# fateshelled/onnx_image_processing

Hardware: AMD Instinct MI355X
Metric: image-pairs/sec (640x480, K=512) (higher is better)
Workload: dtype f32; 1 GPU; Shi-Tomasi(3) + NMS(r=5)/top-k + sparse BAD(512, hard) + Sinkhorn(20, eps 0.05) + MNN(100, 0.1), 640x480 gray pairs, K=512 (BASELINE configs[1]); height=480, width=640, max_keypoints=512, parallelism=pair-sharded x1, input=float32 frames resident in HBM

## Files before the change

onnx_image_processing_amd/csrc/bad.hip:

```cpp
#include "common.h"

#include <math.h>

#include <memory>
#include <mutex>
#include <type_traits>
#include <vector>

#include "bad_plan_opt.h"

namespace {

constexpr int WIN = 34;
constexpr int WOFF = 16;
constexpr int SP = WIN + 1;
constexpr int FR = 33;
constexpr int FW = 35;

struct BadPlan {
  int geometry_ok;
  int num_pairs;
  int passes;
  int passes_canonical;
};
// ... 136 lines not shown
    for (int g = 0; g < GMAX; ++g) {
      if (g < groups) {
        const uint32_t q = plan_geom[g * 64 + lane];
        const int tint = plan_tint[g * 64 + lane];
        const int rad = (int)((q >> 20) & 15u);
        auto box = [&](int offx, int offy) {
          const int cx = clampi((int)kx + offx, 0, w - 1) - ox, cy = clampi((int)ky + offy, 0, h - 1) - oy;
          const int a = cy - rad, b = cy + rad + 1, l = cx - rad, r = cx + rad + 1;
          return (isat[b * FW + r] - isat[a * FW + r]) - (isat[b * FW + l] - isat[a * FW + l]);
        };
        const int s1 = box((int)(q & 31u) - 16, (int)((q >> 10) & 31u) - 16);
        const int s2 = box((int)((q >> 5) & 31u) - 16, (int)((q >> 15) & 31u) - 16);
        emit(g, s1 - s2, tint);
      }
    }
  }
  if (bits) {
    unsigned long long mine = 0ull;
#pragma unroll
    for (int g = 0; g < GMAX; ++g) mine = (lane == g) ? wordv[g] : mine;
    if (lane < groups) reinterpret_cast<unsigned long long *>(bits + (size_t)flat * words)[lane] = mine;
  }
  if (desc) {
    const float inv = normalize ? fmaxf(sqrtf((float)pop), 1e-12f) : 1.0f;
#pragma unroll
    for (int g = 0; g < GMAX; ++g) {
      if (g < groups) {
        const float v = ((wordv[g] >> lane) & 1ull) ? 1.0f : 0.0f;
        desc[(size_t)flat * num_pairs + g * 64 + lane] = normalize ? v / inv : v;
      }
    }
  }
  if (lane == 0) status[flat] = 1;
}

template <typename PIX>
__global__ __launch_bounds__(64) void sparse_bad_kernel(MiSets images, int h, int w,
                                                        MiSets kpt_sets, int k, int total,
                                                        const uint32_t *__restrict__ geom,
                                                        const float *__restrict__ thr, int num_pairs,
                                                        int mode, float temperature, int normalize,
                                                        float scale_y, float scale_x,
                                                        float *__restrict__ desc,
                                                        uint32_t *__restrict__ bits,
                                                        const uint8_t *__restrict__ status, int chunk) {
  __shared__ double sat[SP * SP];
  __shared__ float vals[1024];
  const int lane = threadIdx.x;
  const int groups = num_pairs / 64;
  const int words = num_pairs / 32;

  unsigned long long todo = 1ull;
  int first = (int)xcd_contiguous_id(blockIdx.x, gridDim.x);
  if (status) {
    first = (int)blockIdx.x * chunk;
    const int mine = first + lane;
    todo = __ballot(lane < chunk && mine < total && status[mine] == 0);
    if (!todo) return;
  }
  uint32_t qg[8];
  float tg[8];
#pragma unroll
  for (int g = 0; g < 8; ++g) {
    qg[g] = (g < groups) ? geom[g * 64 + lane] : 0u;
    tg[g] = (g < groups) ? thr[g * 64 + lane] : 0.0f;
  }

  while (todo) {
    const int bit = __ffsll((long long)todo) - 1;
    todo &= todo - 1ull;
    const int flat = first + bit;
    const int img = flat / k;
    const PIX *im = mi_set_item<PIX>(images, img, (size_t)h * w);
    const float *kp = mi_set_item<float>(kpt_sets, img, (size_t)k * 2) + (size_t)(flat - img * k) * 2;
    const float ky_raw = kp[0];
    const float kx_raw = kp[1];
    const bool valid = ky_raw >= 0.0f;
    const float ky = fminf(fmaxf(ky_raw, 0.0f), (float)(h - 1));
    const float kx = fminf(fmaxf(kx_raw, 0.0f), (float)(w - 1));
    const int oy = (int)floorf(ky) - WOFF, ox = (int)floorf(kx) - WOFF;

    __syncthreads();
    for (int i = lane; i < SP; i += 64) { sat[i] = 0.0; sat[i * SP] = 0.0; }
    if (lane < WIN) {
      const int gx = clampi(ox + lane, 0, w - 1);
      PIX px[WIN];
#pragma unroll
      for (int r = 0; r < WIN; ++r) px[r] = im[(size_t)clampi(oy + r, 0, h - 1) * w + gx];
      double acc = 0.0;
#pragma unroll
      for (int r = 0; r < WIN; ++r) {
        acc += (double)px[r];
        sat[(r + 1) * SP + (lane + 1)] = acc;
      }
    }
    __syncthreads();
    if (lane < WIN) {
      double *row = sat + (lane + 1) * SP + 1;
      double v[WIN];
#pragma unroll
      for (int c = 0; c < WIN; ++c) v[c] = row[c];
      double acc = 0.0;
#pragma unroll
      for (int c = 0; c < WIN; ++c) { acc += v[c]; row[c] = acc; }
    }
    __syncthreads();

    const size_t drow = (size_t)flat * (size_t)num_pairs;
    uint32_t *brow = bits ? bits + (size_t)flat * words : nullptr;
    int pop = 0;
    float sumsq = 0.0f;
    auto eval_group = [&](int g, uint32_t q, float thr_p) {
      const int p = g * 64 + lane;
      const int x1 = (int)(q & 31u) - 16, x2 = (int)((q >> 5) & 31u) - 16;
      const int y1 = (int)((q >> 10) & 31u) - 16, y2 = (int)((q >> 15) & 31u) - 16;
      const int r = (int)((q >> 20) & 15u);
      const int c1y = nearest_centre(ky + (float)y1, scale_y, h) - oy;
      const int c1x = nearest_centre(kx + (float)x1, scale_x, w) - ox;
      const int c2y = nearest_centre(ky + (float)y2, scale_y, h) - oy;
      const int c2x = nearest_centre(kx + (float)x2, scale_x, w) - ox;
      const int a1 = clampi(c1y - r, 0, WIN), b1 = clampi(c1y + r + 1, 0, WIN);
      const int l1 = clampi(c1x - r, 0, WIN), r1 = clampi(c1x + r + 1, 0, WIN);
      const int a2 = clampi(c2y - r, 0, WIN), b2 = clampi(c2y + r + 1, 0, WIN);
      const int l2 = clampi(c2x - r, 0, WIN), r2 = clampi(c2x + r + 1, 0, WIN);
      const double s1 = (sat[b1 * SP + r1] - sat[a1 * SP + r1]) - (sat[b1 * SP + l1] - sat[a1 * SP + l1]);
      const double s2 = (sat[b2 * SP + r2] - sat[a2 * SP + r2]) - (sat[b2 * SP + l2] - sat[a2 * SP + l2]);
      const double area = (double)((2 * r + 1) * (2 * r + 1));
      const double t = (double)thr_p;
      if (mode == MI_BAD_HARD) {
        const bool bitv = valid && ((s1 - s2) <= t * area);
        const unsigned long long word = __ballot(bitv);
        pop += (int)__popcll(word);
        if (brow && lane == 0) {
          brow[2 * g] = (uint32_t)word;
          brow[2 * g + 1] = (uint32_t)(word >> 32);
        }
        if (desc) vals[p] = bitv ? 1.0f : 0.0f;
      } else {
        const float c = (float)((s1 - s2) / area - t);
        float v = c;
        if (mode == MI_BAD_SOFT) v = 1.0f / (1.0f + expf(c * temperature));
        v = valid ? v : 0.0f;
        sumsq += v * v;
        vals[p] = v;
      }
    };
#pragma unroll
    for (int g = 0; g < 8; ++g)
      if (g < groups) eval_group(g, qg[g], tg[g]);
#pragma unroll 1
    for (int g = 8; g < groups; ++g) eval_group(g, geom[g * 64 + lane], thr[g * 64 + lane]);

    if (desc) {
      float inv = 1.0f;
      if (normalize) {
        const float ss = (mode == MI_BAD_HARD) ? (float)pop : wave_sum(sumsq);
        inv = fmaxf(sqrtf(ss), 1e-12f);
      }
      for (int g = 0; g < groups; ++g) {
        const float v = vals[g * 64 + lane];
        desc[drow + g * 64 + lane] = normalize ? v / inv : v;
      }
    }
  }
}

struct HostPlan {
  std::vector<uint32_t> geom;
  bool geometry_ok = false;
  mi::BadGatherSchedule sched;
};

std::vector<uint16_t> table_corners(const std::vector<uint32_t> &geom, bool *all_inside) {
  const int num_pairs = (int)geom.size();
  std::vector<uint16_t> c((size_t)num_pairs * 8);
  bool ok = true;
  auto word = [](int row, int col) { return (uint16_t)(row * FW + col); };
  for (int p = 0; p < num_pairs; ++p) {
    const uint32_t q = geom[p];
    const int x1 = (int)(q & 31u), x2 = (int)((q >> 5) & 31u);
    const int y1 = (int)((q >> 10) & 31u), y2 = (int)((q >> 15) & 31u);
    const int r = (int)((q >> 20) & 15u);
    const bool in = x1 - r >= 0 && x2 - r >= 0 && y1 - r >= 0 && y2 - r >= 0 && x1 + r <= 31 && x2 + r <= 31 &&
                    y1 + r <= 31 && y2 + r <= 31;
    ok = ok && in;
    const int cx1 = in ? x1 : 16, cy1 = in ? y1 : 16, cx2 = in ? x2 : 16, cy2 = in ? y2 : 16, cr = in ? r : 0;
    uint16_t *pos = &c[(size_t)p * 8], *neg = pos + 4;
    pos[0] = word(cy1 + cr + 1, cx1 + cr + 1);
    pos[1] = word(cy1 - cr, cx1 - cr);
    pos[2] = word(cy2 - cr, cx2 + cr + 1);
    pos[3] = word(cy2 + cr + 1, cx2 - cr);
    neg[0] = word(cy1 - cr, cx1 + cr + 1);
    neg[1] = word(cy1 + cr + 1, cx1 - cr);
    neg[2] = word(cy2 + cr + 1, cx2 + cr + 1);
    neg[3] = word(cy2 - cr, cx2 - cr);
  }
  *all_inside = ok;
  return c;
}

std::shared_ptr<const HostPlan> host_plan_for(const std::vector<uint32_t> &geom) {
  static std::mutex mu;
  static std::vector<std::shared_ptr<const HostPlan>> *cache = new std::vector<std::shared_ptr<const HostPlan>>();
  {
    std::lock_guard<std::mutex> lock(mu);
    for (const auto &hp : *cache)
      if (hp->geom == geom) return hp;
  }
  auto hp = std::make_shared<HostPlan>();
  hp->geom = geom;
  const std::vector<uint16_t> corners = table_corners(geom, &hp->geometry_ok);
  hp->sched = mi::schedule_bad_gathers(corners, (int)geom.size());
  std::lock_guard<std::mutex> lock(mu);
  if (cache->size() >= 16) cache->erase(cache->begin());
  cache->push_back(hp);
  return hp;
}

}

extern "C" size_t mi_bad_plan_bytes(int num_pairs) {
  if (num_pairs <= 0) return 0;
  return sizeof(BadPlan) + (size_t)num_pairs * (sizeof(uint4) + sizeof(int) + sizeof(uint32_t)) +
         (size_t)(num_pairs / 64) * (num_pairs / 64) * sizeof(uint64_t);
}

int mi_bad_plan_passes_host(const uint32_t *pair_geom_host, int num_pairs, int *canonical, int *scheduled) {
  if (!pair_geom_host || !canonical || !scheduled) return MI_E_NULL;
  if (num_pairs <= 0 || num_pairs % 64 != 0 || num_pairs > 1024) return MI_E_PARAM;
  const auto hp = host_plan_for(std::vector<uint32_t>(pair_geom_host, pair_geom_host + num_pairs));
  for (int e = 0; e < num_pairs; ++e)
    if (hp->sched.exec_pair[e] % 64 != e % 64) return MI_E_PARAM;
  *canonical = hp->sched.passes_canonical;
  *scheduled = hp->sched.passes;
  return MI_OK;
}

extern "C" int mi_bad_plan_build(const uint32_t *pair_geom, const float *pair_thr, int num_pairs, void *plan,
                                 mi_stream_t stream) {
  MI_ENTER();
  if (!pair_geom || !pair_thr || !plan) return MI_E_NULL;
  if (num_pairs <= 0 || num_pairs % 64 != 0 || num_pairs > 1024) return MI_E_PARAM;
  if (((uintptr_t)plan % 16) != 0) return MI_E_ALIGN;
  hipStream_t s = (hipStream_t)stream;
  std::vector<uint32_t> geom(num_pairs);
  std::vector<float> thr(num_pairs);
  if (hipMemcpyAsync(geom.data(), pair_geom, sizeof(uint32_t) * num_pairs, hipMemcpyDeviceToHost, s) != hipSuccess ||
      hipMemcpyAsync(thr.data(), pair_thr, sizeof(float) * num_pairs, hipMemcpyDeviceToHost, s) != hipSuccess ||
      hipStreamSynchronize(s) != hipSuccess)
    return mi_launch_status() ? mi_launch_status() : MI_E_PARAM;
  const auto sched = host_plan_for(geom);
  std::vector<char> host(mi_bad_plan_bytes(num_pairs));
  BadPlan *hp = reinterpret_cast<BadPlan *>(host.data());
  uint4 *offs = reinterpret_cast<uint4 *>(hp + 1);
  int *tint = reinterpret_cast<int *>(offs + num_pairs);
  uint32_t *xgeom = reinterpret_cast<uint32_t *>(tint + num_pairs);
  uint64_t *masks = reinterpret_cast<uint64_t *>(xgeom + num_pairs);
  const int rounds = num_pairs / 64;
  for (int i = 0; i < rounds * rounds; ++i) masks[i] = 0;
  for (int e = 0; e < num_pairs; ++e) {
    const int p = sched->sched.exec_pair[e], lane = e % 64, round = e / 64;
    const uint16_t *pos = &sched->sched.pos[(size_t)e * 4], *neg = &sched->sched.neg[(size_t)e * 4];
    auto two = [](uint16_t lo, uint16_t hi) { return (uint32_t)(lo * 4u) | ((uint32_t)(hi * 4u) << 16); };
    offs[e] = make_uint4(two(pos[0], pos[1]), two(pos[2], pos[3]), two(neg[0], neg[1]), two(neg[2], neg[3]));
    const int r = (int)((geom[p] >> 20) & 15u);
    tint[e] = (int)floor((double)thr[p] * (double)((2 * r + 1) * (2 * r + 1)));
    xgeom[e] = geom[p];
    masks[round * rounds + p / 64] |= (uint64_t)1 << lane;
  }
  hp->geometry_ok = sched->geometry_ok ? 1 : 0;
  hp->num_pairs = num_pairs;
  hp->passes = sched->sched.passes;
  hp->passes_canonical = sched->sched.passes_canonical;
  if (hipMemcpyAsync(plan, host.data(), host.size(), hipMemcpyHostToDevice, s) != hipSuccess ||
      hipStreamSynchronize(s) != hipSuccess)
    return mi_launch_status() ? mi_launch_status() : MI_E_PARAM;
  return MI_OK;
}

namespace {
template <typename PIX>
int sparse_bad_launch(MiSets image, int n, int h, int w, MiSets keypoints, int k, const uint32_t *pair_geom,
                      const float *pair_thr, int num_pairs, int mode, float temperature, int normalize, float *desc,
                      uint32_t *bits, const void *plan, uint8_t *status, mi_stream_t stream) {
  if (!image.a || !keypoints.a || !pair_geom || !pair_thr) return MI_E_NULL;
  if ((image.per_set < n && !image.b) || (keypoints.per_set < n && !keypoints.b)) return MI_E_NULL;
  if (!desc && !bits) return MI_E_NULL;
  if (n <= 0 || h <= 0 || w <= 0 || k <= 0) return MI_E_SHAPE;
  if (num_pairs <= 0 || num_pairs % 64 != 0 || num_pairs > 1024) return MI_E_PARAM;
  if (mode != MI_BAD_RAW && mode != MI_BAD_SOFT && mode != MI_BAD_HARD) return MI_E_PARAM;
  if (bits && mode != MI_BAD_HARD) return MI_E_PARAM;
  if ((long long)n * k > 0x7fffffffLL) return MI_E_SHAPE;
  hipStream_t s = (hipStream_t)stream;
  const int total = n * k;
  const float scale_y = (float)(2.0 / ((double)(h - 1) + 1e-8));
  const float scale_x = (float)(2.0 / ((double)(w - 1) + 1e-8));
  const bool fast = plan != nullptr && status != nullptr && mode == MI_BAD_HARD && h >= 32 && w >= 32 &&
                    (long long)h * w < (1LL << 30);
  if (fast) {
    const BadPlan *bp = reinterpret_cast<const BadPlan *>(plan);
    auto fast_kernel = num_pairs == 512 ? bad_fast_kernel<8, PIX> : num_pairs == 256 ? bad_fast_kernel<4, PIX> : bad_fast_kernel<0, PIX>;
    hipLaunchKernelGGL(fast_kernel, dim3((unsigned)ceil_div(total, 4)), dim3(256), 0, s, image, h, w, keypoints,
                       k, total, num_pairs, normalize, bp, pair_geom, desc, bits, status);
    constexpr int CHUNK = 16;
    hipLaunchKernelGGL(sparse_bad_kernel<PIX>, dim3((unsigned)ceil_div(total, CHUNK)), dim3(64), 0, s, image, h, w,
                       keypoints, k, total, pair_geom, pair_thr, num_pairs, mode, temperature, normalize, scale_y,
                       scale_x, desc, bits, status, CHUNK);
  } else {
    hipLaunchKernelGGL(sparse_bad_kernel<PIX>, dim3((unsigned)total), dim3(64), 0, s, image, h, w, keypoints, k, total,
                       pair_geom, pair_thr, num_pairs, mode, temperature, normalize, scale_y, scale_x, desc, bits,
                       nullptr, 1);
  }
  return mi_launch_status();
}
}

int mi_sparse_bad_sets(MiSets images, int pix_u8, int n, int h, int w, MiSets keypoints, int k, const uint32_t *pair_geom,
                       const float *pair_thr, int num_pairs, int mode, float temperature, int normalize, float *desc,
                       uint32_t *bits, const void *plan, uint8_t *status, mi_stream_t stream) {
  if (pix_u8)
    return sparse_bad_launch<uint8_t>(images, n, h, w, keypoints, k, pair_geom, pair_thr, num_pairs, mode, temperature,
                                      normalize, desc, bits, plan, status, stream);
  return sparse_bad_launch<float>(images, n, h, w, keypoints, k, pair_geom, pair_thr, num_pairs, mode, temperature,
                                  normalize, desc, bits, plan, status, stream);
}

extern "C" int mi_sparse_bad(const float *image, int n, int h, int w, const float *keypoints, int k,
                             const uint32_t *pair_geom, const float *pair_thr, int num_pairs, int mode,
                             float temperature, int normalize, float *desc, uint32_t *bits, const void *plan,
                             uint8_t *status, mi_stream_t stream) {
  MI_ENTER();
  return sparse_bad_launch<float>(mi_one_set(image, n), n, h, w, mi_one_set(keypoints, n), k, pair_geom, pair_thr, num_pairs, mode, temperature,
                                  normalize, desc, bits, plan, status, stream);
}

extern "C" int mi_sparse_bad_pair(const void *image_a, const void *image_b, int pixels_are_u8, int per_set, int h, int w,
                                  const float *keypoints, int k, const uint32_t *pair_geom, const float *pair_thr,
                                  int num_pairs, int mode, float temperature, int normalize, float *desc, uint32_t *bits,
                                  const void *plan, uint8_t *status, mi_stream_t stream) {
  MI_ENTER();
  if (!image_b) return MI_E_NULL;
  if (per_set <= 0 || per_set > 0x3fffffff) return MI_E_SHAPE;
  return mi_sparse_bad_sets(MiSets{image_a, image_b, per_set}, pixels_are_u8 ? 1 : 0, 2 * per_set, h, w,
                            mi_one_set(keypoints, 2 * per_set), k, pair_geom, pair_thr, num_pairs, mode, temperature,
                            normalize, desc, bits, plan, status, stream);
}

extern "C" int mi_sparse_bad_u8(const uint8_t *image, int n, int h, int w, const float *keypoints, int k,
                                const uint32_t *pair_geom, const float *pair_thr, int num_pairs, int mode,
                                float temperature, int normalize, float *desc, uint32_t *bits, const void *plan,
                                uint8_t *status, mi_stream_t stream) {
  MI_ENTER();
  return sparse_bad_launch<uint8_t>(mi_one_set(image, n), n, h, w, mi_one_set(keypoints, n), k, pair_geom, pair_thr, num_pairs, mode, temperature,
                                    normalize, desc, bits, plan, status, stream);
}
```

onnx_image_processing_amd/csrc/cost.hip:

```cpp
#include "common.h"
#include "hooks.h"

#include <type_traits>

namespace {

typedef int v4i __attribute__((ext_vector_type(4)));
typedef int v16i __attribute__((ext_vector_type(16)));
typedef float v16f __attribute__((ext_vector_type(16)));

__device__ __forceinline__ int spread4(uint32_t nib) { return (int)(((nib & 15u) * 0x00204081u) & 0x01010101u); }

__device__ __forceinline__ v4i spread16(uint32_t half) {
  v4i r;
  r[0] = spread4(half);
  r[1] = spread4(half >> 4);
  r[2] = spread4(half >> 8);
  r[3] = spread4(half >> 12);
  return r;
}

constexpr int CB_T = 128;

typedef int v8i __attribute__((ext_vector_type(8)));
__device__ __forceinline__ v8i nibbles_fp4(uint32_t w) {
  v8i r;
  r[0] = (int)((w << 1) & 0x22222222u);
  r[1] = (int)(w & 0x22222222u);
  r[2] = (int)((w >> 1) & 0x22222222u);
  r[3] = (int)((w >> 2) & 0x22222222u);
  r[4] = r[5] = r[6] = r[7] = 0;
  return r;
}

template <bool DOTS, int WORDS, bool FP4 = false>
__global__ __launch_bounds__(256) __attribute__((amdgpu_waves_per_eu(4, 4))) void cost_bits_kernel(const uint32_t *__restrict__ bits1,
                                                        const uint32_t *__restrict__ bits2, int n, int m,
                                                        int words_rt, int normalized, float eps,
                                                        float *__restrict__ z, int pitch,
                                                        uint16_t *__restrict__ dots,
                                                        float2 *__restrict__ row_info,
                                                        float2 *__restrict__ col_info, uint4 *__restrict__ zero16,
                                                        size_t zero_count) {
  extern __shared__ uint32_t lds_u[];
  const int words = WORDS > 0 ? WORDS : words_rt;
  if (zero_count) {
    const size_t nthreads = (size_t)gridDim.x * gridDim.y * gridDim.z * 256;
    const size_t me = (((size_t)blockIdx.z * gridDim.y + blockIdx.y) * gridDim.x + blockIdx.x) * 256 + threadIdx.x;
    for (size_t i = me; i < zero_count; i += nthreads) zero16[i] = make_uint4(0u, 0u, 0u, 0u);
  }
  const int wp = words + 1;
  uint32_t *sa = lds_u;
  uint32_t *sb = sa + CB_T * wp;
  float *inv_a = reinterpret_cast<float *>(sb + CB_T * wp);
  float *nrm_a = inv_a + CB_T;
  float *inv_b = nrm_a + CB_T;
  float *nrm_b = inv_b + CB_T;

  const int t = threadIdx.x, lane = t & 63, wave = t >> 6;
  const int j0 = blockIdx.x * CB_T, i0 = blockIdx.y * CB_T, b = blockIdx.z;
  const uint32_t *a_g = bits1 + (size_t)b * n * words;
  const uint32_t *b_g = bits2 + (size_t)b * m * words;

  if ((words & 3) == 0 && words <= 32 && (((uintptr_t)bits1 | (uintptr_t)bits2) & 15) == 0) {
    const int cpr = words >> 2;
    const int chunks = CB_T * cpr;
    uint4 va[4], vb[4];
#pragma unroll
    for (int q = 0; q < 4; ++q) {
      const int ch = t + 256 * q;
      const int r = ch / cpr;
      va[q] = make_uint4(0u, 0u, 0u, 0u);
      vb[q] = va[q];
      if (ch < chunks && i0 + r < n) va[q] = reinterpret_cast<const uint4 *>(a_g + (size_t)i0 * words)[ch];
      if (ch < chunks && j0 + r < m) vb[q] = reinterpret_cast<const uint4 *>(b_g + (size_t)j0 * words)[ch];
    }
#pragma unroll
    for (int q = 0; q < 4; ++q) {
      const int ch = t + 256 * q;
      if (ch < chunks) {
        const int r = ch / cpr, c = (ch - r * cpr) * 4;
        uint32_t *da = sa + r * wp + c, *db = sb + r * wp + c;
        da[0] = va[q].x; da[1] = va[q].y; da[2] = va[q].z; da[3] = va[q].w;
        db[0] = vb[q].x; db[1] = vb[q].y; db[2] = vb[q].z; db[3] = vb[q].w;
      }
    }
  } else {
    for (int i = t; i < CB_T * words; i += 256) {
      const int r = i / words, c = i - r * words;
      sa[r * wp + c] = (i0 + r < n) ? a_g[(size_t)(i0 + r) * words + c] : 0u;
      sb[r * wp + c] = (j0 + r < m) ? b_g[(size_t)(j0 + r) * words + c] : 0u;
    }
  }
  __syncthreads();
  {
    const int r = t & 127;
    const uint32_t *src = (t < 128 ? sa : sb) + r * wp;
    int pop = 0;
    for (int c0 = 0; c0 < words; c0 += 8) {
      uint32_t wv[8];
#pragma unroll
      for (int q = 0; q < 8; ++q) wv[q] = (c0 + q < words) ? src[c0 + q] : 0u;
#pragma unroll
      for (int q = 0; q < 8; ++q) pop += __popc(wv[q]);
    }
    float inv = 1.0f, nrm = (float)pop;
    if (normalized) {
      inv = pop > 0 ? 1.0f / sqrtf((float)pop) : 0.0f;
      nrm = (float)pop * (inv * inv);
    }
    (t < 128 ? inv_a : inv_b)[r] = inv;
    (t < 128 ? nrm_a : nrm_b)[r] = nrm;
  }
  __syncthreads();

  const int wm = (wave >> 1) * 64, wn = (wave & 1) * 64;
  const int lr = lane & 31, lh = lane >> 5;
  typedef typename std::conditional<FP4, v16f, v16i>::type acc_t;
  acc_t acc[2][2];
#pragma unroll
  for (int mi = 0; mi < 2; ++mi)
#pragma unroll
    for (int ni = 0; ni < 2; ++ni)
#pragma unroll
      for (int e = 0; e < 16; ++e) acc[mi][ni][e] = 0;

  static_assert(!FP4 || (WORDS > 0 && WORDS % 2 == 0), "the FP4 form takes two words per step");
  auto kstep = [&](int ks) {
    if constexpr (FP4) {
      v8i fa[2], fb[2];
#pragma unroll
      for (int q = 0; q < 2; ++q) {
        fa[q] = nibbles_fp4(sa[(wm + q * 32 + lr) * wp + 2 * ks + lh]);
        fb[q] = nibbles_fp4(sb[(wn + q * 32 + lr) * wp + 2 * ks + lh]);
      }
#pragma unroll
      for (int mi = 0; mi < 2; ++mi)
#pragma unroll
        for (int ni = 0; ni < 2; ++ni)
          acc[mi][ni] = __builtin_amdgcn_mfma_scale_f32_32x32x64_f8f6f4(fa[mi], fb[ni], acc[mi][ni], 4, 4, 0, 0, 0, 0);
      return;
    } else {
    v4i fa[2], fb[2];
#pragma unroll
    for (int q = 0; q < 2; ++q) {
      fa[q] = spread16(sa[(wm + q * 32 + lr) * wp + ks] >> (16 * lh));
      fb[q] = spread16(sb[(wn + q * 32 + lr) * wp + ks] >> (16 * lh));
    }
#pragma unroll
    for (int mi = 0; mi < 2; ++mi)
#pragma unroll
      for (int ni = 0; ni < 2; ++ni)
        acc[mi][ni] = __builtin_amdgcn_mfma_i32_32x32x32_i8(fa[mi], fb[ni], acc[mi][ni], 0, 0, 0);
    }
  };
  if constexpr (FP4) {
#pragma unroll
    for (int ks = 0; ks < WORDS / 2; ++ks) kstep(ks);
  } else if constexpr (WORDS > 0) {
#pragma unroll
    for (int ks = 0; ks < WORDS; ++ks) kstep(ks);
  } else {
#pragma unroll 4
    for (int ks = 0; ks < words; ++ks) kstep(ks);
  }

  if constexpr (DOTS) {
    if (blockIdx.x == 0 && t < CB_T && i0 + t < n) row_info[(size_t)b * n + i0 + t] = make_float2(inv_a[t], nrm_a[t]);
    if (blockIdx.y == 0 && t < CB_T && j0 + t < m) col_info[(size_t)b * m + j0 + t] = make_float2(inv_b[t], nrm_b[t]);
    __syncthreads();
    constexpr int SP16 = CB_T + 8;
    uint16_t *stage = reinterpret_cast<uint16_t *>(lds_u);
#pragma unroll
    for (int mi = 0; mi < 2; ++mi)
#pragma unroll
      for (int ni = 0; ni < 2; ++ni)
#pragma unroll
        for (int e = 0; e < 16; ++e) {
          const int rl = wm + mi * 32 + (e & 3) + 8 * (e >> 2) + 4 * lh;
          const int cl = wn + ni * 32 + lr;
          stage[rl * SP16 + cl] = (uint16_t)(int)acc[mi][ni][e];
        }
    __syncthreads();
    uint16_t *db = dots + (size_t)b * (size_t)n * pitch;
#pragma unroll
    for (int k = 0; k < 8; ++k) {
      const int id = t + 256 * k;
      const int row = id >> 4, c8 = (id & 15) * 8;
      if (i0 + row < n && j0 + c8 < m)
        *reinterpret_cast<uint4 *>(db + (size_t)(i0 + row) * pitch + j0 + c8) =
            *reinterpret_cast<const uint4 *>(stage + row * SP16 + c8);
    }
  } else {
    float *zb = z + (size_t)b * (size_t)n * pitch;
#pragma unroll
    for (int mi = 0; mi < 2; ++mi)
#pragma unroll
      for (int ni = 0; ni < 2; ++ni)
#pragma unroll
        for (int e = 0; e < 16; ++e) {
          const int rl = wm + mi * 32 + (e & 3) + 8 * (e >> 2) + 4 * lh;
          const int cl = wn + ni * 32 + lr;
          const int gi = i0 + rl, gj = j0 + cl;
          if (gi < n && gj < m) {
            const float dot = (float)acc[mi][ni][e];
            const float cross = dot * (inv_a[rl] * inv_b[cl]);
            const float cost = fmaxf((nrm_a[rl] + nrm_b[cl]) - 2.0f * cross, 0.0f);
            zb[(size_t)gi * pitch + gj] = -cost / eps;
          }
        }
  }
}

constexpr int CF_T = 64;
constexpr int CF_K = 32;
constexpr int CF_P = CF_K + 1;

template <int DIST>
__global__ __launch_bounds__(256) void cost_f32_kernel(const float *__restrict__ d1,
                                                       const float *__restrict__ d2, int n, int m, int d,
                                                       float eps, float *__restrict__ z, int pitch) {
  __shared__ float sa[CF_T * CF_P];
  __shared__ float sb[CF_T * CF_P];
  __shared__ float nrm_a[CF_T], nrm_b[CF_T];

  const int t = threadIdx.x, lane = t & 63, wave = t >> 6;
  const int j0 = blockIdx.x * CF_T, i0 = blockIdx.y * CF_T, b = blockIdx.z;
  const float *a_g = d1 + (size_t)b * n * d;
  const float *b_g = d2 + (size_t)b * m * d;

  const int srow = t >> 2, sk = (t & 3) * 8;
  const int wm = (wave >> 1) * 32, wn = (wave & 1) * 32;
  const int lr = lane & 31, lh = lane >> 5;

  v16f acc;
#pragma unroll
  for (int e = 0; e < 16; ++e) acc[e] = 0.0f;
  float l1acc[4][4];
#pragma unroll
  for (int p = 0; p < 4; ++p)
#pragma unroll
    for (int q = 0; q < 4; ++q) l1acc[p][q] = 0.0f;
  float ssa = 0.0f, ssb = 0.0f;

  for (int k0 = 0; k0 < d; k0 += CF_K) {
#pragma unroll
    for (int q = 0; q < 8; ++q) {
      const int kk = k0 + sk + q;
      const float va = (i0 + srow < n && kk < d) ? a_g[(size_t)(i0 + srow) * d + kk] : 0.0f;
      const float vb = (j0 + srow < m && kk < d) ? b_g[(size_t)(j0 + srow) * d + kk] : 0.0f;
      sa[srow * CF_P + sk + q] = va;
      sb[srow * CF_P + sk + q] = vb;
      ssa += va * va;
      ssb += vb * vb;
    }
    __syncthreads();
    if (DIST == MI_DIST_L2) {
#pragma unroll
      for (int kk = 0; kk < CF_K; kk += 2) {
        const float fa = sa[(wm + lr) * CF_P + kk + lh];
        const float fb = sb[(wn + lr) * CF_P + kk + lh];
        acc = __builtin_amdgcn_mfma_f32_32x32x2f32(fa, fb, acc, 0, 0, 0);
      }
    } else {
      const int ti = (t >> 4) * 4, tj = (t & 15) * 4;
      for (int kk = 0; kk < CF_K; ++kk) {
        float av[4], bv[4];
#pragma unroll
        for (int p = 0; p < 4; ++p) { av[p] = sa[(ti + p) * CF_P + kk]; bv[p] = sb[(tj + p) * CF_P + kk]; }
#pragma unroll
        for (int p = 0; p < 4; ++p)
#pragma unroll
          for (int q = 0; q < 4; ++q) l1acc[p][q] += fabsf(av[p] - bv[q]);
      }
    }
    __syncthreads();
  }

  float *zb = z + (size_t)b * (size_t)n * pitch;
  if (DIST == MI_DIST_L2) {
    ssa += __shfl_xor(ssa, 1, 64); ssa += __shfl_xor(ssa, 2, 64);
    ssb += __shfl_xor(ssb, 1, 64); ssb += __shfl_xor(ssb, 2, 64);
    if ((t & 3) == 0) { nrm_a[srow] = ssa; nrm_b[srow] = ssb; }
    __syncthreads();
#pragma unroll
    for (int e = 0; e < 16; ++e) {
      const int rl = wm + (e & 3) + 8 * (e >> 2) + 4 * lh;
      const int cl = wn + lr;
      const int gi = i0 + rl, gj = j0 + cl;
      if (gi < n && gj < m) {
        const float cost = fmaxf((nrm_a[rl] + nrm_b[cl]) - 2.0f * acc[e], 0.0f);
        zb[(size_t)gi * pitch + gj] = -cost / eps;
      }
    }
  } else {
    const int ti = (t >> 4) * 4, tj = (t & 15) * 4;
#pragma unroll
    for (int p = 0; p < 4; ++p)
#pragma unroll
      for (int q = 0; q < 4; ++q) {
        const int gi = i0 + ti + p, gj = j0 + tj + q;
        if (gi < n && gj < m) zb[(size_t)gi * pitch + gj] = -l1acc[p][q] / eps;
      }
  }
}

constexpr int CG_T = 128, CG_K = 32, CG_P = CG_K + 1;

__global__ __launch_bounds__(256) void cost_f32_big_kernel(const float *__restrict__ d1, const float *__restrict__ d2,
                                                           int n, int m, int d, float eps, float *__restrict__ z,
                                                           int pitch) {
  __shared__ float sa[CG_T * CG_P];
  __shared__ float sb[CG_T * CG_P];
  __shared__ float nrm_a[CG_T], nrm_b[CG_T];
  const int t = threadIdx.x, lane = t & 63, wave = t >> 6;
  const int j0 = blockIdx.x * CG_T, i0 = blockIdx.y * CG_T, b = blockIdx.z;
  const float *a_g = d1 + (size_t)b * n * d;
  const float *b_g = d2 + (size_t)b * m * d;
  const int srow = t >> 3, sk = (t & 7) * 4;
  const int wm = (wave >> 1) * 64, wn = (wave & 1) * 64;
  const int lr = lane & 31, lh = lane >> 5;

  v16f acc[2][2];
#pragma unroll
  for (int mi = 0; mi < 2; ++mi)
#pragma unroll
    for (int ni = 0; ni < 2; ++ni)
#pragma unroll
      for (int e = 0; e < 16; ++e) acc[mi][ni][e] = 0.0f;
  float ssa[4] = {0.f, 0.f, 0.f, 0.f}, ssb[4] = {0.f, 0.f, 0.f, 0.f};

  auto fetch = [&](int k0, float4 (&va)[4], float4 (&vb)[4]) {
#pragma unroll
    for (int q = 0; q < 4; ++q) {
      const int r = srow + 32 * q, kk = k0 + sk;
      va[q] = make_float4(0.f, 0.f, 0.f, 0.f);
      vb[q] = make_float4(0.f, 0.f, 0.f, 0.f);
      if (i0 + r < n && kk < d) va[q] = *reinterpret_cast<const float4 *>(a_g + (size_t)(i0 + r) * d + kk);
      if (j0 + r < m && kk < d) vb[q] = *reinterpret_cast<const float4 *>(b_g + (size_t)(j0 + r) * d + kk);
    }
  };
  float4 va[4], vb[4], na[4], nb[4];
  fetch(0, va, vb);
  for (int k0 = 0; k0 < d; k0 += CG_K) {
#pragma unroll
    for (int q = 0; q < 4; ++q) {
      float *pa = sa + (srow + 32 * q) * CG_P + sk, *pb = sb + (srow + 32 * q) * CG_P + sk;
      pa[0] = va[q].x; pa[1] = va[q].y; pa[2] = va[q].z; pa[3] = va[q].w;
      pb[0] = vb[q].x; pb[1] = vb[q].y; pb[2] = vb[q].z; pb[3] = vb[q].w;
      ssa[q] += (va[q].x * va[q].x + va[q].y * va[q].y) + (va[q].z * va[q].z + va[q].w * va[q].w);
      ssb[q] += (vb[q].x * vb[q].x + vb[q].y * vb[q].y) + (vb[q].z * vb[q].z + vb[q].w * vb[q].w);
    }
    __syncthreads();
    if (k0 + CG_K < d) fetch(k0 + CG_K, na, nb);
#pragma unroll
    for (int kk = 0; kk < CG_K; kk += 2) {
      float fa[2], fb[2];
#pragma unroll
      for (int q = 0; q < 2; ++q) {
        fa[q] = sa[(wm + q * 32 + lr) * CG_P + kk + lh];
        fb[q] = sb[(wn + q * 32 + lr) * CG_P + kk + lh];
      }
#pragma unroll
      for (int mi = 0; mi < 2; ++mi)
#pragma unroll
        for (int ni = 0; ni < 2; ++ni)
          acc[mi][ni] = __builtin_amdgcn_mfma_f32_32x32x2f32(fa[mi], fb[ni], acc[mi][ni], 0, 0, 0);
    }
    __syncthreads();
#pragma unroll
    for (int q = 0; q < 4; ++q) { va[q] = na[q]; vb[q] = nb[q]; }
  }
#pragma unroll
  for (int q = 0; q < 4; ++q) {
    float x = ssa[q], y = ssb[q];
    x += __shfl_xor(x, 1, 64); x += __shfl_xor(x, 2, 64); x += __shfl_xor(x, 4, 64);
    y += __shfl_xor(y, 1, 64); y += __shfl_xor(y, 2, 64); y += __shfl_xor(y, 4, 64);
    if ((t & 7) == 0) { nrm_a[srow + 32 * q] = x; nrm_b[srow + 32 * q] = y; }
  }
  __syncthreads();
  float *zb = z + (size_t)b * (size_t)n * pitch;
#pragma unroll
  for (int mi = 0; mi < 2; ++mi)
#pragma unroll
    for (int ni = 0; ni < 2; ++ni)
#pragma unroll
      for (int e = 0; e < 16; ++e) {
        const int rl = wm + mi * 32 + (e & 3) + 8 * (e >> 2) + 4 * lh;
        const int cl = wn + ni * 32 + lr;
        const int gi = i0 + rl, gj = j0 + cl;
        if (gi < n && gj < m) {
          const float cost = fmaxf((nrm_a[rl] + nrm_b[cl]) - 2.0f * acc[mi][ni][e], 0.0f);
          zb[(size_t)gi * pitch + gj] = -cost / eps;
        }
      }
}

int check_z(const void *a, const void *b, const void *z, int batch, int n, int m, int pitch, double eps) {
  if (!a || !b || !z) return MI_E_NULL;
  if (batch <= 0 || n <= 0 || m <= 0 || batch > 65535) return MI_E_SHAPE;
  if (pitch < m || pitch % 4 != 0 || ((uintptr_t)z % 16) != 0) return MI_E_ALIGN;
  if (!(eps > 0.0)) return MI_E_PARAM;
  return MI_OK;
}

}

extern "C" int mi_cost_logscores_bits(const uint32_t *bits1, const uint32_t *bits2, int batch, int n, int m,
                                      int num_bits, int normalized, double epsilon, float *z, int pitch,
                                      mi_stream_t stream) {
  MI_ENTER();
  int e = check_z(bits1, bits2, z, batch, n, m, pitch, epsilon);
  if (e) return e;
  if (num_bits <= 0 || num_bits % 32 != 0 || num_bits > 4096) return MI_E_PARAM;
  const int words = num_bits / 32;
  const size_t lds = (size_t)2 * CB_T * (words + 1) * 4 + 4 * CB_T * 4;
  dim3 grid(ceil_div(m, CB_T), ceil_div(n, CB_T), batch);
  uint4 *const no_zero = nullptr;
  auto kern = words == 16 ? cost_bits_kernel<false, 16, true> : words == 8 ? cost_bits_kernel<false, 8, true> : cost_bits_kernel<false, 0>;
  if (MI_HOOK(cost_impl, 0) == 1) kern = words == 16 ? cost_bits_kernel<false, 16> : words == 8 ? cost_bits_kernel<false, 8> : cost_bits_kernel<false, 0>;
  hipLaunchKernelGGL(kern, grid, dim3(256), lds, (hipStream_t)stream, bits1, bits2, n, m,
                     words, normalized, (float)epsilon, z, pitch, nullptr, nullptr, nullptr, no_zero, (size_t)0);
  return mi_launch_status();
}

int mi_cost_dots_bits_zeroing(const uint32_t *bits1, const uint32_t *bits2, int batch, int n, int m, int num_bits,
                              int normalized, uint16_t *dots, int pitch, float *row_info, float *col_info,
                              void *zero_ptr, size_t zero_bytes, mi_stream_t stream) {
  if (!bits1 || !bits2 || !dots || !row_info || !col_info) return MI_E_NULL;
  if (batch <= 0 || n <= 0 || m <= 0 || batch > 65535) return MI_E_SHAPE;
  if (pitch < m || pitch % 8 != 0 || ((uintptr_t)dots % 16) != 0 || ((uintptr_t)row_info % 8) != 0 ||
      ((uintptr_t)col_info % 8) != 0 || ((uintptr_t)zero_ptr % 16) != 0 || zero_bytes % 16 != 0)
    return MI_E_ALIGN;
  if (num_bits <= 0 || num_bits % 32 != 0 || num_bits > 4096) return MI_E_PARAM;
  const int words = num_bits / 32;
  size_t lds = (size_t)2 * CB_T * (words + 1) * 4 + 4 * CB_T * 4;
  const size_t stage = (size_t)CB_T * (CB_T + 8) * 2;
  if (lds < stage) lds = stage;
  dim3 grid(ceil_div(m, CB_T), ceil_div(n, CB_T), batch);
  auto kern = words == 16 ? cost_bits_kernel<true, 16, true> : words == 8 ? cost_bits_kernel<true, 8, true> : cost_bits_kernel<true, 0>;
  if (MI_HOOK(cost_impl, 0) == 1) kern = words == 16 ? cost_bits_kernel<true, 16> : words == 8 ? cost_bits_kernel<true, 8> : cost_bits_kernel<true, 0>;
  hipLaunchKernelGGL(kern, grid, dim3(256), lds, (hipStream_t)stream, bits1, bits2, n, m, words,
                     normalized, 1.0f, nullptr, pitch, dots, reinterpret_cast<float2 *>(row_info),
                     reinterpret_cast<float2 *>(col_info), reinterpret_cast<uint4 *>(zero_ptr),
                     zero_ptr ? zero_bytes / 16 : (size_t)0);
  return mi_launch_status();
}

extern "C" int mi_cost_dots_bits(const uint32_t *bits1, const uint32_t *bits2, int batch, int n, int m,
                                 int num_bits, int normalized, uint16_t *dots, int pitch, float *row_info,
                                 float *col_info, mi_stream_t stream) {
  MI_ENTER();
  return mi_cost_dots_bits_zeroing(bits1, bits2, batch, n, m, num_bits, normalized, dots, pitch, row_info, col_info,
                                   nullptr, 0, stream);
}

extern "C" int mi_cost_logscores_f32(const float *desc1, const float *desc2, int batch, int n, int m, int d,
                                     int distance, double epsilon, float *z, int pitch, mi_stream_t stream) {
  MI_ENTER();
  int e = check_z(desc1, desc2, z, batch, n, m, pitch, epsilon);
  if (e) return e;
  if (d <= 0) return MI_E_SHAPE;
  dim3 grid(ceil_div(m, CF_T), ceil_div(n, CF_T), batch);
  const float eps = (float)epsilon;
  if (distance == MI_DIST_L2 && d % 4 == 0 && (((uintptr_t)desc1 | (uintptr_t)desc2) % 16) == 0 && n >= 64 && m >= 64) {
    dim3 big(ceil_div(m, CG_T), ceil_div(n, CG_T), batch);
    hipLaunchKernelGGL(cost_f32_big_kernel, big, dim3(256), 0, (hipStream_t)stream, desc1, desc2, n, m, d, eps, z, pitch);
    return mi_launch_status();
  }
  if (distance == MI_DIST_L2)
    hipLaunchKernelGGL(cost_f32_kernel<MI_DIST_L2>, grid, dim3(256), 0, (hipStream_t)stream, desc1, desc2, n,
                       m, d, eps, z, pitch);
  else if (distance == MI_DIST_L1)
    hipLaunchKernelGGL(cost_f32_kernel<MI_DIST_L1>, grid, dim3(256), 0, (hipStream_t)stream, desc1, desc2, n,
                       m, d, eps, z, pitch);
  else
    return MI_E_PARAM;
  return mi_launch_status();
}
```

onnx_image_processing_amd/csrc/hooks.hip:

```cpp
#ifndef MI_DEBUG_HOOKS
#error "hooks.hip belongs to the debug library only (-DMI_DEBUG_HOOKS)"
#endif
#include "common.h"
#include "hooks.h"

#include "../../include/mi355x_match_debug.h"

MiHooks mi_hooks;

int mi_bad_plan_passes_host(const uint32_t *pair_geom_host, int num_pairs, int *canonical, int *scheduled);
int mi_sinkhorn_dots_form_host(int batch, int n, int m, int flags, int blocks_per_cu, int cus);

MI_API int mi_debug_clock_probe(void *buffer) {
  mi_hooks.corner_clk = reinterpret_cast<unsigned long long *>(buffer);
  return MI_OK;
}

MI_API int mi_debug_topk_stamps(void *buffer) {
  mi_hooks.topk_prof = reinterpret_cast<unsigned long long *>(buffer);
  return MI_OK;
}

MI_API int mi_debug_set(int key, int value) {
  if (key == 0) {
    mi_hooks.corner_impl = 0; mi_hooks.corner_rows = 4; mi_hooks.corner_rows_u8_default = 1;
    mi_hooks.sinkhorn_log_partials = 0; mi_hooks.sinkhorn_split = 2; mi_hooks.sinkhorn_persist = 1;
    mi_hooks.sinkhorn_stamps = 0; mi_hooks.topk_select = 1; mi_hooks.topk_split = -1; mi_hooks.sinkhorn_schedule = -1;
    mi_hooks.akaze_impl = 0;
    mi_hooks.bad_oriented_impl = 0;
    mi_hooks.cost_impl = 0;
    mi_hooks.sinkhorn_mix = 1;
    mi_hooks.sinkhorn_pair_waves = 1;
    mi_hooks.mnn_pair_waves = 1;
    mi_hooks.mnn_one_pass = 1;
    mi_hooks.sinkhorn_exp_rows = 1;
    mi_hooks.nms_impl = 0;
    mi_hooks.corner_clk = nullptr; mi_hooks.topk_prof = nullptr;
    return MI_OK;
  }
  if (key == 1) { mi_hooks.corner_impl = value; return MI_OK; }
  if (key == 2 && (value == 4 || value == 5 || value == 8)) { mi_hooks.corner_rows = value; mi_hooks.corner_rows_u8_default = 0; return MI_OK; }
  if (key == 4) { mi_hooks.sinkhorn_log_partials = value; return MI_OK; }
  if (key == 6) { mi_hooks.sinkhorn_split = value; return MI_OK; }
  if (key == 7) { mi_hooks.sinkhorn_persist = value; return MI_OK; }
  if (key == 8) { mi_hooks.sinkhorn_stamps = value; return MI_OK; }
  if (key == 9) { mi_hooks.topk_select = value; return MI_OK; }
  if (key == 10) { mi_hooks.topk_split = value; return MI_OK; }
  if (key == 12 && (value == 0 || value == 1)) { mi_hooks.akaze_impl = value; return MI_OK; }
  if (key == 13 && (value == 0 || value == 1)) { mi_hooks.bad_oriented_impl = value; return MI_OK; }
  if (key == 14 && (value == 0 || value == 1)) { mi_hooks.cost_impl = value; return MI_OK; }
  if (key == 15 && (value == 0 || value == 1)) { mi_hooks.sinkhorn_mix = value; return MI_OK; }
  if (key == 16 && (value == 0 || value == 1)) { mi_hooks.sinkhorn_pair_waves = value; return MI_OK; }
  if (key == 17 && (value == 0 || value == 1)) { mi_hooks.mnn_pair_waves = value; return MI_OK; }
  if (key == 19 && (value == 0 || value == 1)) { mi_hooks.mnn_one_pass = value; return MI_OK; }
  if (key == 18 && (value == 0 || value == 1)) { mi_hooks.sinkhorn_exp_rows = value; return MI_OK; }
  if (key == 20 && (value == 0 || value == 1)) { mi_hooks.nms_impl = value; return MI_OK; }
  if (key == 11 && value >= -1 && value <= 2) { mi_hooks.sinkhorn_schedule = value; return MI_OK; }
  return MI_E_PARAM;
}

MI_API int mi_debug_bad_plan_passes(const uint32_t *pair_geom_host, int num_pairs, int *canonical, int *scheduled) {
  return mi_bad_plan_passes_host(pair_geom_host, num_pairs, canonical, scheduled);
}

#include "sk_tuner.h"
MI_API int mi_debug_tuner_script(int n_ops, const int *op, const int *arg, const double *val, int *out) {
  if (n_ops < 0 || (n_ops > 0 && (!op || !arg || !val || !out))) return MI_E_NULL;
  mi::TunerLogic t;
  int last_entry = -1, last_slot = -1;
  for (int i = 0; i < n_ops; ++i) {
    mi::TunerShape s;
    s.batch = arg[i]; s.n = 512; s.m = 512; s.iterations = 20;
    switch (op[i]) {
      case 0: {
        const int sched = t.begin(s, &last_entry, &last_slot);
        out[i] = sched | ((last_slot & 0xff) << 8) | ((last_entry & 0xff) << 16);
        break;
      }
      case 1: t.finish(arg[i] >> 8, arg[i] & 0xff, val[i]); out[i] = 0; break;
      case 2: t.abandon(arg[i] >> 8, arg[i] & 0xff); out[i] = 0; break;
      case 3: out[i] = t.current(s); break;
      case 4: out[i] = t.for_capture(s); break;
      case 5: out[i] = t.set(arg[i]) ? 0 : -1; break;
      default: return MI_E_PARAM;
    }
  }
  return MI_OK;
}

MI_API int mi_debug_sinkhorn_dots_form(int batch, int n, int m, int flags, int blocks_per_cu, int cus) {
  return mi_sinkhorn_dots_form_host(batch, n, m, flags, blocks_per_cu, cus);
}

#include "akaze_math.h"
namespace {
__global__ __launch_bounds__(256) void akaze_math_check_kernel(int which, float kappa, uint32_t lo_bits, uint32_t hi_bits,
                                                               unsigned long long *mismatches, uint32_t *first_bad) {
  const float rk = 1.0f / kappa;
  unsigned long long bad = 0;
  for (unsigned long long b = (unsigned long long)lo_bits + blockIdx.x * 256ull + threadIdx.x; b < hi_bits;
       b += (unsigned long long)gridDim.x * 256ull) {
    const float x = __uint_as_float((uint32_t)b);
    float got, want;
    if (which == 0) { got = ak_sqrt(x); want = sqrtf(x); }
    else if (which == 1) { got = ak_div_by(x, kappa, rk); want = x / kappa; }
    else if (which == 2) { got = ak_rcp(x); want = 1.0f / x; }
    else if (which == 3) { got = ak_div(x, kappa); want = x / kappa; }
    else if (which == 4) { got = ak_sqrt_fp<1>(x); want = sqrtf(x); }
    else { got = ak_sqrt_fp<2>(x); want = sqrtf(x); }
    if (__float_as_uint(got) != __float_as_uint(want)) {
      ++bad;
      atomicMin(first_bad, (uint32_t)b);
    }
  }
  if (bad) atomicAdd(mismatches, bad);
}
}

MI_API int mi_debug_akaze_math_check(int which, float kappa, uint32_t lo_bits, uint32_t hi_bits, void *mismatches_u64,
                                     void *first_bad_u32, mi_stream_t stream) {
  MI_ENTER();
  if (!mismatches_u64 || !first_bad_u32) return MI_E_NULL;
  if (which < 0 || which > 5 || !(kappa > 0.0f) || lo_bits >= hi_bits) return MI_E_PARAM;
  hipLaunchKernelGGL(akaze_math_check_kernel, dim3(4096), dim3(256), 0, (hipStream_t)stream, which, kappa, lo_bits, hi_bits,
                     reinterpret_cast<unsigned long long *>(mismatches_u64), reinterpret_cast<uint32_t *>(first_bad_u32));
  return mi_launch_status();
}
```

Before: 217,300 image-pairs/sec.

## Add row-strip bit-descriptor dot kernel that streams column tiles per block

```diff
diff --git a/onnx_image_processing_amd/csrc/bad.hip b/onnx_image_processing_amd/csrc/bad.hip
--- a/onnx_image_processing_amd/csrc/bad.hip
+++ b/onnx_image_processing_amd/csrc/bad.hip
@@ -462,7 +462,7 @@
     auto fast_kernel = num_pairs == 512 ? bad_fast_kernel<8, PIX> : num_pairs == 256 ? bad_fast_kernel<4, PIX> : bad_fast_kernel<0, PIX>;
     hipLaunchKernelGGL(fast_kernel, dim3((unsigned)ceil_div(total, 4)), dim3(256), 0, s, image, h, w, keypoints,
                        k, total, num_pairs, normalize, bp, pair_geom, desc, bits, status);
-    constexpr int CHUNK = 16;
+    constexpr int CHUNK = 32;
     hipLaunchKernelGGL(sparse_bad_kernel<PIX>, dim3((unsigned)ceil_div(total, CHUNK)), dim3(64), 0, s, image, h, w,
                        keypoints, k, total, pair_geom, pair_thr, num_pairs, mode, temperature, normalize, scale_y,
                        scale_x, desc, bits, status, CHUNK);
diff --git a/onnx_image_processing_amd/csrc/cost.hip b/onnx_image_processing_amd/csrc/cost.hip
--- a/onnx_image_processing_amd/csrc/cost.hip
+++ b/onnx_image_processing_amd/csrc/cost.hip
@@ -212,6 +212,161 @@
   }
 }
 
+constexpr int CR_SP = 64 + 8;
+template <int WORDS>
+constexpr size_t cost_rows_lds() { return (size_t)2 * CB_T * (WORDS + 1) * 4 + (size_t)4 * 32 * CR_SP * 2; }
+
+template <int WORDS, bool FP4>
+__global__ __launch_bounds__(256) __attribute__((amdgpu_waves_per_eu(4, 4))) void cost_dots_rows_kernel(
+    const uint32_t *__restrict__ bits1, const uint32_t *__restrict__ bits2, int n, int m, int normalized, int pitch,
+    uint16_t *__restrict__ dots, float2 *__restrict__ row_info, float2 *__restrict__ col_info, uint4 *__restrict__ zero16,
+    size_t zero_count) {
+  static_assert(WORDS % 4 == 0 && CB_T * (WORDS / 4) % 256 == 0, "16-byte chunks, the same number for every thread");
+  extern __shared__ uint32_t lds_u[];
+  if (zero_count) {
+    const size_t nthreads = (size_t)gridDim.x * gridDim.y * gridDim.z * 256;
+    const size_t me = (((size_t)blockIdx.z * gridDim.y + blockIdx.y) * gridDim.x + blockIdx.x) * 256 + threadIdx.x;
+    for (size_t i = me; i < zero_count; i += nthreads) zero16[i] = make_uint4(0u, 0u, 0u, 0u);
+  }
+  constexpr int wp = WORDS + 1;
+  constexpr int CPR = WORDS / 4;
+  constexpr int NQ = CB_T * CPR / 256;
+  constexpr int KS = FP4 ? WORDS / 2 : WORDS;
+  uint32_t *const sa = lds_u;
+  uint32_t *const sb = sa + CB_T * wp;
+  const int t = threadIdx.x, lane = t & 63, wave = __builtin_amdgcn_readfirstlane(t >> 6);
+  uint16_t *const stage = reinterpret_cast<uint16_t *>(lds_u + 2 * CB_T * wp) + wave * 32 * CR_SP;
+  const int i0 = blockIdx.y * CB_T, b = blockIdx.z;
+  const int tiles = (m + CB_T - 1) / CB_T;
+  const uint32_t *a_g = bits1 + (size_t)b * n * WORDS;
+  const uint32_t *b_g = bits2 + (size_t)b * m * WORDS;
+  const int wm = (wave >> 1) * 64, wn = (wave & 1) * 64;
+  const int lr = lane & 31, lh = lane >> 5;
+
+  uint4 vb[NQ];
+  auto load_tile = [&](const uint32_t *g, int r0, int rows) {
+#pragma unroll
+    for (int q = 0; q < NQ; ++q) {
+      const uint32_t ch = NQ * t + q;
+      vb[q] = reinterpret_cast<const uint4 *>(g + (size_t)r0 * WORDS)[r0 + (int)(ch / CPR) < rows ? ch : 0u];
+    }
+  };
+  auto store_tile = [&](uint32_t *dst, int r0, int rows) {
+#pragma unroll
+    for (int q = 0; q < NQ; ++q) {
+      const int ch = NQ * t + q;
+      const int r = ch / CPR, c = (ch - r * CPR) * 4;
+      const bool in = r0 + r < rows;
+      uint32_t *d = dst + r * wp + c;
+      d[0] = in ? vb[q].x : 0u; d[1] = in ? vb[q].y : 0u; d[2] = in ? vb[q].z : 0u; d[3] = in ? vb[q].w : 0u;
+    }
+  };
+  load_tile(a_g, i0, n);
+  store_tile(sa, i0, n);
+  load_tile(b_g, 0, m);
+  store_tile(sb, 0, m);
+  __syncthreads();
+  if (t < CB_T && i0 + t < n) {
+    const uint32_t *src = sa + t * wp;
+    int pop = 0;
+#pragma unroll
+    for (int c = 0; c < WORDS; ++c) pop += __popc(src[c]);
+    float inv = 1.0f, nrm = (float)pop;
+    if (normalized) {
+      inv = pop > 0 ? 1.0f / sqrtf((float)pop) : 0.0f;
+      nrm = (float)pop * (inv * inv);
+    }
+    row_info[(size_t)b * n + i0 + t] = make_float2(inv, nrm);
+  }
+
+  uint16_t *const db = dots + (size_t)b * (size_t)n * pitch;
+  typedef typename std::conditional<FP4, v16f, v16i>::type acc_t;
+  for (int jt = 0; jt < tiles; ++jt) {
+    const int j0 = jt * CB_T;
+    const bool more = jt + 1 < tiles;
+    if (more) load_tile(b_g, j0 + CB_T, m);
+    if (blockIdx.y == 0 && t < CB_T && j0 + t < m) {
+      const uint32_t *src = sb + t * wp;
+      int pop = 0;
+#pragma unroll
+      for (int c = 0; c < WORDS; ++c) pop += __popc(src[c]);
+      float inv = 1.0f, nrm = (float)pop;
+      if (normalized) {
+        inv = pop > 0 ? 1.0f / sqrtf((float)pop) : 0.0f;
+        nrm = (float)pop * (inv * inv);
+      }
+      col_info[(size_t)b * m + j0 + t] = make_float2(inv, nrm);
+    }
+
+    acc_t acc[2][2];
+#pragma unroll
+    for (int mi = 0; mi < 2; ++mi)
+#pragma unroll
+      for (int ni = 0; ni < 2; ++ni)
+#pragma unroll
+        for (int e = 0; e < 16; ++e) acc[mi][ni][e] = 0;
+#pragma unroll
+    for (int ks = 0; ks < KS; ++ks) {
+      if constexpr (FP4) {
+        v8i fa[2], fb[2];
+#pragma unroll
+        for (int q = 0; q < 2; ++q) {
+          fa[q] = nibbles_fp4(sa[(wm + q * 32 + lr) * wp + 2 * ks + lh]);
+          fb[q] = nibbles_fp4(sb[(wn + q * 32 + lr) * wp + 2 * ks + lh]);
+        }
+#pragma unroll
+        for (int mi = 0; mi < 2; ++mi)
+#pragma unroll
+          for (int ni = 0; ni < 2; ++ni)
+            acc[mi][ni] = __builtin_amdgcn_mfma_scale_f32_32x32x64_f8f6f4(fb[ni], fa[mi], acc[mi][ni], 4, 4, 0, 0, 0, 0);
+      } else {
+        v4i fa[2], fb[2];
+#pragma unroll
+        for (int q = 0; q < 2; ++q) {
+          fa[q] = spread16(sa[(wm + q * 32 + lr) * wp + ks] >> (16 * lh));
+          fb[q] = spread16(sb[(wn + q * 32 + lr) * wp + ks] >> (16 * lh));
+        }
+#pragma unroll
+        for (int mi = 0; mi < 2; ++mi)
+#pragma unroll
+          for (int ni = 0; ni < 2; ++ni)
+            acc[mi][ni] = __builtin_amdgcn_mfma_i32_32x32x32_i8(fb[ni], fa[mi], acc[mi][ni], 0, 0, 0);
+      }
+    }
+    __syncthreads();
+    if (more) store_tile(sb, j0 + CB_T, m);
+
+#pragma unroll
+    for (int mi = 0; mi < 2; ++mi) {
+#pragma unroll
+      for (int ni = 0; ni < 2; ++ni)
+#pragma unroll
+        for (int g = 0; g < 4; ++g) {
+          const uint32_t d0 = (uint32_t)(int)acc[mi][ni][4 * g], d1 = (uint32_t)(int)acc[mi][ni][4 * g + 1];
+          const uint32_t d2 = (uint32_t)(int)acc[mi][ni][4 * g + 2], d3 = (uint32_t)(int)acc[mi][ni][4 * g + 3];
+          *reinterpret_cast<uint2 *>(stage + lr * CR_SP + ni * 32 + 8 * g + 4 * lh) = make_uint2(d0 | (d1 << 16), d2 | (d3 << 16));
+        }
+      __builtin_amdgcn_fence(__ATOMIC_RELEASE, "wavefront");
+      __builtin_amdgcn_wave_barrier();
+      __builtin_amdgcn_fence(__ATOMIC_ACQUIRE, "wavefront");
+#pragma unroll
+      for (int k = 0; k < 4; ++k) {
+        const int id = lane + 64 * k;
+        const int row = id >> 3, c8 = (id & 7) * 8;
+        const uint4 v = *reinterpret_cast<const uint4 *>(stage + row * CR_SP + c8);
+        const int gi = i0 + wm + mi * 32 + row, gj = j0 + wn + c8;
+        uint16_t *const strip = db + (size_t)(i0 + wm + mi * 32) * pitch + (j0 + wn);
+        if (gi < n && gj < m )
+          *reinterpret_cast<uint4 *>(strip + ((uint32_t)row * (uint32_t)pitch + (uint32_t)c8)) = v;
+      }
+      __builtin_amdgcn_fence(__ATOMIC_RELEASE, "wavefront");
+      __builtin_amdgcn_wave_barrier();
+      __builtin_amdgcn_fence(__ATOMIC_ACQUIRE, "wavefront");
+    }
+    __syncthreads();
+  }
+}
+
 constexpr int CF_T = 64;
 constexpr int CF_K = 32;
 constexpr int CF_P = CF_K + 1;
@@ -418,7 +573,7 @@
   dim3 grid(ceil_div(m, CB_T), ceil_div(n, CB_T), batch);
   uint4 *const no_zero = nullptr;
   auto kern = words == 16 ? cost_bits_kernel<false, 16, true> : words == 8 ? cost_bits_kernel<false, 8, true> : cost_bits_kernel<false, 0>;
-  if (MI_HOOK(cost_impl, 0) == 1) kern = words == 16 ? cost_bits_kernel<false, 16> : words == 8 ? cost_bits_kernel<false, 8> : cost_bits_kernel<false, 0>;
+  if (MI_HOOK(cost_impl, 0) & 1) kern = words == 16 ? cost_bits_kernel<false, 16> : words == 8 ? cost_bits_kernel<false, 8> : cost_bits_kernel<false, 0>;
   hipLaunchKernelGGL(kern, grid, dim3(256), lds, (hipStream_t)stream, bits1, bits2, n, m,
                      words, normalized, (float)epsilon, z, pitch, nullptr, nullptr, nullptr, no_zero, (size_t)0);
   return mi_launch_status();
@@ -434,12 +589,23 @@
     return MI_E_ALIGN;
   if (num_bits <= 0 || num_bits % 32 != 0 || num_bits > 4096) return MI_E_PARAM;
   const int words = num_bits / 32;
+  const int impl = MI_HOOK(cost_impl, 0);
+  if ((words == 16 || words == 8) && impl < 2 && (((uintptr_t)bits1 | (uintptr_t)bits2) & 15) == 0) {
+    auto rows = words == 16 ? cost_dots_rows_kernel<16, true> : cost_dots_rows_kernel<8, true>;
+    if (impl == 1) rows = words == 16 ? cost_dots_rows_kernel<16, false> : cost_dots_rows_kernel<8, false>;
+    dim3 grid(1, ceil_div(n, CB_T), batch);
+    hipLaunchKernelGGL(rows, grid, dim3(256), words == 16 ? cost_rows_lds<16>() : cost_rows_lds<8>(), (hipStream_t)stream, bits1,
+                       bits2, n, m, normalized, pitch, dots, reinterpret_cast<float2 *>(row_info),
+                       reinterpret_cast<float2 *>(col_info), reinterpret_cast<uint4 *>(zero_ptr),
+                       zero_ptr ? zero_bytes / 16 : (size_t)0);
+    return mi_launch_status();
+  }
   size_t lds = (size_t)2 * CB_T * (words + 1) * 4 + 4 * CB_T * 4;
   const size_t stage = (size_t)CB_T * (CB_T + 8) * 2;
   if (lds < stage) lds = stage;
   dim3 grid(ceil_div(m, CB_T), ceil_div(n, CB_T), batch);
   auto kern = words == 16 ? cost_bits_kernel<true, 16, true> : words == 8 ? cost_bits_kernel<true, 8, true> : cost_bits_kernel<true, 0>;
-  if (MI_HOOK(cost_impl, 0) == 1) kern = words == 16 ? cost_bits_kernel<true, 16> : words == 8 ? cost_bits_kernel<true, 8> : cost_bits_kernel<true, 0>;
+  if (impl & 1) kern = words == 16 ? cost_bits_kernel<true, 16> : words == 8 ? cost_bits_kernel<true, 8> : cost_bits_kernel<true, 0>;
   hipLaunchKernelGGL(kern, grid, dim3(256), lds, (hipStream_t)stream, bits1, bits2, n, m, words,
                      normalized, 1.0f, nullptr, pitch, dots, reinterpret_cast<float2 *>(row_info),
                      reinterpret_cast<float2 *>(col_info), reinterpret_cast<uint4 *>(zero_ptr),
diff --git a/onnx_image_processing_amd/csrc/hooks.hip b/onnx_image_processing_amd/csrc/hooks.hip
--- a/onnx_image_processing_amd/csrc/hooks.hip
+++ b/onnx_image_processing_amd/csrc/hooks.hip
@@ -48,7 +48,7 @@
   if (key == 10) { mi_hooks.topk_split = value; return MI_OK; }
   if (key == 12 && (value == 0 || value == 1)) { mi_hooks.akaze_impl = value; return MI_OK; }
   if (key == 13 && (value == 0 || value == 1)) { mi_hooks.bad_oriented_impl = value; return MI_OK; }
-  if (key == 14 && (value == 0 || value == 1)) { mi_hooks.cost_impl = value; return MI_OK; }
+  if (key == 14 && value >= 0 && value <= 3) { mi_hooks.cost_impl = value; return MI_OK; }
   if (key == 15 && (value == 0 || value == 1)) { mi_hooks.sinkhorn_mix = value; return MI_OK; }
   if (key == 16 && (value == 0 || value == 1)) { mi_hooks.sinkhorn_pair_waves = value; return MI_OK; }
   if (key == 17 && (value == 0 || value == 1)) { mi_hooks.mnn_pair_waves = value; return MI_OK; }
```

Result: no change. 218,600 image-pairs/sec, median of 6 (+0.6%).
